# wahn/rs_pbrt

Measured on AMD Instinct MI355X. Metric: Mpath-samples/sec (whole node), higher is better.
Workload: dtype f32; 1 GPU; synthetic 1000000-triangle soup, path depth 8, sobol 256 spp, 1024x1024; tiles=16x16 tiles in Morton order dealt round-robin to the ranks (tile_chunk 1), film_reduce=none (1 GPU), devices_visible=1

## Files before the change

rs_pbrt_amd/csrc/launch_trace.h:

```cpp
uint32_t hinted_grid(uint32_t hint, uint32_t full, uint32_t per_block) {
    if (hint == 0xffffffffu) return full;
    const uint64_t need = (2ull * hint + per_block - 1) / per_block + 1;
    return (uint32_t)std::min<uint64_t>(full, need);
}
bool trace_can_overflow(const rspt_scene_s* s) {
    const size_t which = env_size("RSPT_TRACE_KERNEL", 2);
    const size_t rows = std::min<size_t>(env_size("RSPT_W4_SPILL_ROWS", RSPT_W4_SPILL), RSPT_W4_SPILL);
    return s->has_instances || (s->has_alpha && !s->w4_ok) || !(which >= 2 && s->w4_ok) || RSPT_W4_LDS + rows < RSPT_W4_MAX_STACK;
}
uint32_t trace_grid() { return grid_for((uint32_t)env_size("RSPT_TRACE_BLOCKS_PER_CU", 5)); }
#ifndef RSPT_PW_CHUNK_CAMERA_DEFAULT
#define RSPT_PW_CHUNK_CAMERA_DEFAULT 1024
#endif
#ifndef RSPT_PW_REFILL_CAMERA_DEFAULT
#define RSPT_PW_REFILL_CAMERA_DEFAULT 48
#endif
#ifndef RSPT_PW_ENTER
#define RSPT_PW_ENTER 24
#endif
struct TraceCall {
    const uint32_t* queue = nullptr; const uint32_t* count_ptr = nullptr; uint32_t count_imm = 0;
    uint32_t* cursor = nullptr;
    const rspt_ray* ra = nullptr; const rspt_ray* rb = nullptr;
    float4* oa = nullptr; float4* ob = nullptr;
    uint32_t* occ = nullptr;
    rspt_hit* hits = nullptr;
    unsigned long long* counters = nullptr; uint32_t* xcd_cursors = nullptr;
    int lane = 0;
    bool count = false;
    bool camera_launch = false;
    int force_any_q = -1;
    int force_camera_pk = -1;
    uint32_t* inst_out = nullptr;
    uint32_t queue_hint = 0xffffffffu;
};
struct TracePre { hipStream_t stream; uint32_t* ovf; uint2* spill; uint32_t pgrid; int refill, leaf; uint32_t chunk; };
TracePre trace_pre(const TraceCall& c, bool camera) {
    TracePre p; p.stream = c.lane ? g.stream2 : g.stream;
    p.ovf = g.ovf + (c.lane ? 2 * g.ovf_cap / 3 : 0);
    p.spill = g.spill + (c.lane ? g.spill_threads * RSPT_W4_SPILL : 0);
    p.pgrid = hinted_grid(c.queue_hint, pw_grid(), RSPT_PW_BLOCK);
    p.refill = (int)(camera ? env_size("RSPT_PW_REFILL_CAMERA", RSPT_PW_REFILL_CAMERA_DEFAULT) : env_size("RSPT_PW_REFILL", RSPT_PW_REFILL));
    p.leaf = (int)(camera ? env_size("RSPT_PW_LEAF_CAMERA", env_size("RSPT_PW_LEAF", RSPT_PW_LEAF)) : env_size("RSPT_PW_LEAF", RSPT_PW_LEAF));
    p.chunk = (uint32_t)std::min<size_t>(std::max<size_t>((camera ? env_size("RSPT_PW_CHUNK_CAMERA", RSPT_PW_CHUNK_CAMERA_DEFAULT) : env_size("RSPT_PW_CHUNK", RSPT_PW_CHUNK)) & ~(size_t)63, 64), 1u << 20);
    return p;
}
bool camera_packet_ok(const rspt_scene_s* s, size_t which, const uint32_t* xcur) {
    return which >= 2 && s->w4_ok && s->w4 && s->leaf_boxes && !s->has_instances && !s->has_alpha && !s->has_spheres && !(s->w4_root & RSPT_REF_LEAF) &&
           env_size("RSPT_W4_SHAPE", RSPT_W4_SHAPE_DEFAULT) == 0 && !xcur;
}
bool camera_packet_wanted(const rspt_scene_s* s, const TraceCall& c) {
    if (c.force_camera_pk >= 0) return c.force_camera_pk != 0;
    const char* e = getenv("RSPT_CAMERA_PACKET");
    if (e && *e) return atoi(e) != 0;
    return c.camera_launch && s->camera_pk_choice > 0;
}
template <bool ANY, int OUT_MODE, bool INST, bool ALPHA>
void launch_trace_v(uint32_t grid, const rspt_scene_s* s, const TraceCall& c, uint32_t* xcur) {
    const SceneDev& sc = s->dev;
    const size_t which = env_size("RSPT_TRACE_KERNEL", 2);
    const TracePre p = trace_pre(c, c.camera_launch);
    uint32_t* hi = (INST && OUT_MODE == 0 && !ANY) ? (c.inst_out ? c.inst_out : g.hit_inst) : nullptr;
    const bool special = INST || ALPHA;
    const bool anim_w4 = s->has_animated && s->w4_ok && which >= 2 && env_size("RSPT_ANIM_W4", 1) != 0 && env_size("RSPT_INSTANCE_KERNEL", 1) != 0;
    const bool slow = c.count || which == 0 || (s->has_animated && !anim_w4) || (special && (!s->w4_ok || env_size("RSPT_INSTANCE_KERNEL", 1) == 0));
    if (slow) {
        if (INST && s->has_animated)
            hipLaunchKernelGGL((k_trace<ANY, OUT_MODE, false, true, ALPHA, true>), dim3(grid), dim3(RSPT_TRACE_BLOCK), 0, p.stream, sc, s->tex, c.queue, c.count_ptr, c.count_imm, c.ra, c.rb, c.oa, c.ob, c.occ, c.hits, c.counters, hi);
        else if (c.count)
            hipLaunchKernelGGL((k_trace<ANY, OUT_MODE, true, INST, ALPHA>), dim3(grid), dim3(RSPT_TRACE_BLOCK), 0, p.stream, sc, s->tex, c.queue, c.count_ptr, c.count_imm, c.ra, c.rb, c.oa, c.ob, c.occ, c.hits, c.counters, hi);
        else
            hipLaunchKernelGGL((k_trace<ANY, OUT_MODE, false, INST, ALPHA>), dim3(grid), dim3(RSPT_TRACE_BLOCK), 0, p.stream, sc, s->tex, c.queue, c.count_ptr, c.count_imm, c.ra, c.rb, c.oa, c.ob, c.occ, c.hits, c.counters, hi);
        return;
    }
    const uint32_t pw_chunk = p.chunk | (env_size("RSPT_PW_ADAPT", 1) != 0 ? 0u : 1u);
    grid = hinted_grid(c.queue_hint, grid, RSPT_TRACE_BLOCK);
    uint32_t* n_overflow = c.cursor + 2;
    const uint32_t spill_rows = (uint32_t)std::min<size_t>(env_size("RSPT_W4_SPILL_ROWS", RSPT_W4_SPILL), RSPT_W4_SPILL);
    if constexpr (INST) {
        if (anim_w4) {
            const int pw_enter = (int)std::min<size_t>(std::max<size_t>(env_size("RSPT_PW_ENTER", RSPT_PW_ENTER), 1), 64);
            auto go = [&](auto kern) {
                hipLaunchKernelGGL(kern, dim3(p.pgrid), dim3(RSPT_PW_BLOCK), 0, p.stream, sc, s->tex, s->w4, s->big_leaves, s->w4_root, c.queue, c.count_ptr, c.count_imm, c.cursor,
                                   c.ra, c.rb, c.oa, c.ob, c.occ, c.hits, n_overflow, p.ovf, p.spill, spill_rows, p.refill, (p.leaf & 0xff) | (pw_enter << 8), s->w4_top, hi, xcur, pw_chunk);
            };
            if constexpr (ALPHA) { if (s->alpha_simple) go(k_trace_w4<ANY, OUT_MODE, true, 2, true>); else go(k_trace_w4<ANY, OUT_MODE, true, 1, true>); }
            else go(k_trace_w4<ANY, OUT_MODE, true, 0, true>);
            hipLaunchKernelGGL((k_trace_fixup<ANY, OUT_MODE, true, ALPHA, true>), dim3(grid), dim3(RSPT_TRACE_BLOCK), 0, p.stream, sc, s->tex, n_overflow, p.ovf, c.ra, c.rb, c.oa, c.ob, c.occ, c.hits, hi);
            return;
        }
    }
    if constexpr (ANY && !INST && !ALPHA) {
        const char* q_env = getenv("RSPT_ANY_Q");
        const bool use_q = c.force_any_q >= 0 ? c.force_any_q != 0 : (q_env && *q_env ? atoi(q_env) != 0 : s->any_q_choice > 0);
        if (use_q && which >= 2 && s->w4q && !(s->w4_root & RSPT_REF_LEAF) && c.ra == c.rb && env_size("RSPT_W4_SHAPE", RSPT_W4_SHAPE_DEFAULT) == 0 && !xcur && spill_rows == RSPT_W4_SPILL) {
            hipLaunchKernelGGL((k_trace_w4q<OUT_MODE>), dim3(p.pgrid), dim3(RSPT_PW_BLOCK), 0, p.stream, sc, s->w4q, s->big_leaves, s->w4_root, c.queue, c.count_ptr, c.count_imm, c.cursor,
                               c.ra, c.occ, c.hits, reinterpret_cast<uint32_t*>(p.spill), p.refill, p.leaf, s->w4_top,
                               pw_chunk | (env_size("RSPT_ANY_Q_LATE", 1) != 0 ? 2u : 0u) , s->leaf_boxes);
            return;
        }
    }
    if constexpr (!ANY && !INST && !ALPHA) {
        if (camera_packet_wanted(s, c) && camera_packet_ok(s, which, xcur)) {
            const uint32_t kgrid = hinted_grid(c.queue_hint, grid_for((uint32_t)std::min<size_t>(std::max<size_t>(env_size("RSPT_PK_BLOCKS_PER_CU", 6), 1), 8)), RSPT_PW_BLOCK);
            hipLaunchKernelGGL((k_trace_w4pk<OUT_MODE>), dim3(kgrid), dim3(RSPT_PW_BLOCK), 0, p.stream, sc, s->w4, s->big_leaves, s->w4_root, c.queue, c.count_ptr, c.count_imm, c.cursor,
                               c.ra, c.rb, c.oa, c.ob, c.hits, pw_chunk, s->leaf_boxes);
            return;
        }
    }
    if constexpr (!INST && !ALPHA) {
        const size_t shape = which >= 2 && s->w4_ok ? env_size("RSPT_W4_SHAPE", RSPT_W4_SHAPE_DEFAULT) : 0;
        if (shape == 1 || shape == 2) {
            auto go = [&](auto kern, uint32_t block, uint32_t topcap, uint32_t per_cu) -> bool {
                const size_t lds = (size_t)8 * RSPT_W4_LDS * block + (size_t)112 * topcap;
                static bool attr_set[2][2][2][3] = {};
                bool& done = attr_set[ANY ? 1 : 0][OUT_MODE ? 1 : 0][0][shape];
                static bool attr_bad[2][2][2][3] = {};
                bool& bad = attr_bad[ANY ? 1 : 0][OUT_MODE ? 1 : 0][0][shape];
                if (!done) { bad = hipFuncSetAttribute(reinterpret_cast<const void*>(kern), hipFuncAttributeMaxDynamicSharedMemorySize, (int)lds) != hipSuccess; (void)hipGetLastError(); done = true; }
                if (bad) return false;
                const uint32_t bgrid = hinted_grid(c.queue_hint, grid_for(per_cu), block);
                hipLaunchKernelGGL(kern, dim3(bgrid), dim3(block), lds, p.stream, sc, s->tex, s->w4, s->big_leaves, s->w4_root, c.queue, c.count_ptr, c.count_imm, c.cursor,
                                   c.ra, c.rb, c.oa, c.ob, c.occ, c.hits, n_overflow, p.ovf, p.spill, spill_rows, p.refill, p.leaf, s->w4_top, hi, xcur, pw_chunk);
                return true;
            };
            const bool launched = shape == 1 ? go(k_trace_w4<ANY, OUT_MODE, false, 0, false, 1024, 512>, 1024u, 512u, 1u) : go(k_trace_w4<ANY, OUT_MODE, false, 0, false, 512, 256>, 512u, 256u, 2u);
            if (launched) {
                if (trace_can_overflow(s))
                    hipLaunchKernelGGL((k_trace_fixup<ANY, OUT_MODE, INST, ALPHA>), dim3(grid), dim3(RSPT_TRACE_BLOCK), 0, p.stream, sc, s->tex, n_overflow, p.ovf, c.ra, c.rb, c.oa, c.ob, c.occ, c.hits, hi);
                return;
            }
        }
    }
    if (ALPHA && s->alpha_simple)
        hipLaunchKernelGGL((k_trace_w4<ANY, OUT_MODE, INST, ALPHA ? 2 : 0>), dim3(p.pgrid), dim3(RSPT_PW_BLOCK), 0, p.stream, sc, s->tex, s->w4, s->big_leaves, s->w4_root, c.queue, c.count_ptr, c.count_imm, c.cursor,
                           c.ra, c.rb, c.oa, c.ob, c.occ, c.hits, n_overflow, p.ovf, p.spill, spill_rows, p.refill, p.leaf, s->w4_top, hi, xcur, pw_chunk);
    else if (special || (which >= 2 && s->w4_ok))
        hipLaunchKernelGGL((k_trace_w4<ANY, OUT_MODE, INST, ALPHA ? 1 : 0>), dim3(p.pgrid), dim3(RSPT_PW_BLOCK), 0, p.stream, sc, s->tex, s->w4, s->big_leaves, s->w4_root, c.queue, c.count_ptr, c.count_imm, c.cursor,
                           c.ra, c.rb, c.oa, c.ob, c.occ, c.hits, n_overflow, p.ovf, p.spill, spill_rows, p.refill, p.leaf, s->w4_top, hi, xcur, pw_chunk);
// ... 64 lines not shown
```

rs_pbrt_amd/csrc/render_schedules.h:

```cpp
#define RSPT_LANE_ROWS(WH) {{k_lane_dl<false, false, false, WH>, k_lane_dl<false, true, false, WH>}, {k_lane_dl<true, false, false, WH>, k_lane_dl<true, true, false, WH>}, {k_lane_dl<true, false, true, WH>, k_lane_dl<true, true, true, WH>}}
typedef void (*LaneKernel)(SceneDev, TexTables, LightDistDev, RenderDev, Batch, PathBuf, const uint32_t*, LaneDesc);
const LaneKernel g_lane_dl[2][3][2] = {RSPT_LANE_ROWS(false), RSPT_LANE_ROWS(true)};
#undef RSPT_LANE_ROWS
int RenderRun::build_claimed_rows(uint32_t* n_claimed) {
    LightLazy lz;
    HIP_TRY(hipMemcpyAsync(g.look, ld_lazy->lazy, sizeof lz, hipMemcpyDeviceToHost, g.stream));
    HIP_TRY(hipStreamSynchronize(g.stream));
    memcpy(&lz, g.look, sizeof lz);
    *n_claimed = lz.n_new;
    if (lz.overflow) return fail(RSPT_E_NOMEM, "spatial light distribution: more than %u voxels were touched; raise RSPT_LIGHT_TABLE_POOL_BYTES", lz.max_rows);
    if (lz.n_new == 0) return RSPT_OK;
    const uint32_t lgrid = grid_for(4);
    hipLaunchKernelGGL(k_ld_contrib_list, dim3(lgrid), dim3(256), 0, g.stream, s->dev, ld.nvox[0], ld.nvox[1], ld.nvox[2], ld_lazy->lazy, ld_lazy->new_list, ld_lazy->func);
    hipLaunchKernelGGL(k_ld_build_list, dim3(lgrid), dim3(256), 0, g.stream, s->dev.n_lights, ld_lazy->lazy, ld_lazy->new_list, ld_lazy->func, ld_lazy->cdf, ld_lazy->func_int, ld_lazy->table);
    hipLaunchKernelGGL(k_ld_commit, dim3(1), dim3(1), 0, g.stream, ld_lazy->lazy);
    return RSPT_OK;
}
int RenderRun::tune_any(uint32_t batch_n, TraceCall c) {
    if (!s->w4q || s->any_q_choice >= 0 || getenv("RSPT_ANY_Q") || counters || batch_n < (1u << 22) || env_size("RSPT_ANY_Q_TUNE", 1) == 0) return 0;
    hipEvent_t t0 = get_event(n_ev++), t1 = get_event(n_ev++), t2 = get_event(n_ev++);
    if (hipEventRecord(t0, g.stream) != hipSuccess) return RSPT_E_HIP;
    c.force_any_q = 0;
    launch_trace<true, 0>(tgrid, s, c);
    (void)hipEventRecord(t1, g.stream);
    (void)hipMemsetAsync(c.cursor, 0, sizeof(uint32_t), g.stream);
    c.force_any_q = 1;
    launch_trace<true, 0>(tgrid, s, c);
    (void)hipEventRecord(t2, g.stream);
    if (hipEventSynchronize(t2) != hipSuccess) return RSPT_E_HIP;
    float ms_plain = 0.0f, ms_q = 0.0f;
    (void)hipEventElapsedTime(&ms_plain, t0, t1);
    (void)hipEventElapsedTime(&ms_q, t1, t2);
    s->any_q_choice = ms_q < ms_plain ? 1 : 0;
    if (getenv("RSPT_VERBOSE")) fprintf(stderr, "rspt: shadow rays of this scene: k_trace_w4<any> %.2f ms, k_trace_w4q %.2f ms on the same launch -> %s\n", ms_plain, ms_q, s->any_q_choice ? "the quantised records" : "the plain records");
    return 1;
}
int RenderRun::tune_camera(uint32_t batch_n, TraceCall c) {
    if (s->camera_pk_choice >= 0 || getenv("RSPT_CAMERA_PACKET") || counters || d->integrator != RSPT_INTEGRATOR_PATH || batch_n < (1u << 22) || env_size("RSPT_CAMERA_PACKET_TUNE", 1) == 0) return 0;
    if (!camera_packet_ok(s, env_size("RSPT_TRACE_KERNEL", 2), (c.xcd_cursors && env_size("RSPT_XCD_DEAL", 0) != 0) ? c.xcd_cursors : nullptr)) return 0;
    hipEvent_t t0 = get_event(n_ev++), t1 = get_event(n_ev++), t2 = get_event(n_ev++);
    if (hipEventRecord(t0, g.stream) != hipSuccess) return RSPT_E_HIP;
    c.force_camera_pk = 0;
    launch_trace<false, 0>(tgrid, s, c);
    (void)hipEventRecord(t1, g.stream);
    (void)hipMemsetAsync(c.cursor, 0, sizeof(uint32_t), g.stream);
    c.force_camera_pk = 1;
    launch_trace<false, 0>(tgrid, s, c);
    (void)hipEventRecord(t2, g.stream);
    if (hipEventSynchronize(t2) != hipSuccess) return RSPT_E_HIP;
    float ms_w4 = 0.0f, ms_pk = 0.0f;
    (void)hipEventElapsedTime(&ms_w4, t0, t1);
    (void)hipEventElapsedTime(&ms_pk, t1, t2);
    s->camera_pk_choice = ms_pk < ms_w4 ? 1 : 0;
    if (getenv("RSPT_VERBOSE")) fprintf(stderr, "rspt: camera rays of this scene: k_trace_w4 %.2f ms, k_trace_w4pk %.2f ms on the same launch -> %s\n", ms_w4, ms_pk, s->camera_pk_choice ? "64-ray packets" : "per-lane walks");
    return 1;
}
int RenderRun::batch_volpath(const Batch& bt, uint32_t& it) {
    int rc;
    const uint32_t dgrid = grid_for(4);
    const uint32_t null_passes = (uint32_t)env_size("RSPT_NULL_PASSES", 1024);
    const uint32_t vnd = std::min(1024u, 5u + 10u * (d->max_depth + 2u) + 128u) + 8u;
    if ((size_t)vnd * sob_bits * 4 > 64 * 1024) return fail(RSPT_E_UNSUPPORTED, "volpath: max_depth %u x %u index bits exceed the LDS Sobol' table", d->max_depth, sob_bits);
    const uint32_t vlimit = halton ? vol_dim_limit : std::min(1024u, vnd - 8u);
    hipLaunchKernelGGL(k_vol_init, dim3((bt.n + 255) / 256), dim3(256), 0, g.stream, g.vol, bt.n);
    uint32_t live = bt.n;
    for (uint32_t pass = 0; live > 0; pass++) {
        const int par = pass & 1;
        QueueCounts* cur = &g.cnt[par];
        QueueCounts* nxt = &g.cnt[par ^ 1];
        HIP_TRY(hipMemsetAsync(nxt, 0, sizeof(QueueCounts), g.stream));
        HIP_TRY(hipMemsetAsync(&g.cnt[2], 0, sizeof(QueueCounts), g.stream));
        ev_open(0, 0);
        launch_trace<false, 0>(tgrid, s, closest_call(g.pb, g.q[par][1], &cur->closest, &cur->cursor_closest, counters));
        ev_close(0, 0);
        trace_launches++;
        vol_rays += live;
        ev_open(2, 0);
        if (s->has_textures) hipLaunchKernelGGL(k_texture, dim3(dgrid), dim3(256), 0, g.stream, s->dev, s->tex, rd, g.pb, g.q[par][1], &cur->closest, (const uint32_t*)nullptr, (const BinInfo*)nullptr);
        if (ld.lazy) HIP_TRY(hipMemsetAsync(&cur->active, 0, sizeof(uint32_t), g.stream));
        hipLaunchKernelGGL(s->has_dynamic ? k_vol_shade<true> : k_vol_shade<false>, dim3(dgrid), dim3(256), halton ? 0 : vnd * sob_bits * sizeof(uint32_t), g.stream, s->dev, ld, rd, g.pb, g.vol, g.q[par][1], &cur->closest,
                           g.q[par ^ 1][1], &nxt->closest, g.q[0][2], &g.cnt[2].closest, vlimit, vnd, sob_bits, ld.lazy ? g.q[par][0] : (uint32_t*)nullptr, &cur->active);
        for (uint32_t round = 0; ld.lazy; round++) {
            uint32_t claimed = 0;
            if ((rc = build_claimed_rows(&claimed))) return rc;
            HIP_TRY(hipMemcpyAsync(g.look, cur, sizeof(QueueCounts), hipMemcpyDeviceToHost, g.stream));
            HIP_TRY(hipStreamSynchronize(g.stream));
            const uint32_t n_retry = g.look[0].active;
// ... 378 lines not shown
```

rs_pbrt_amd/csrc/trace_packet.h:

```cpp
#pragma once
#include "trace_w4.h"

namespace rspt {

#define RSPT_PK_WAVES (RSPT_PW_BLOCK / 64)
#ifdef RSPT_PK_OCC
#define RSPT_PK_ATTR __attribute__((amdgpu_waves_per_eu(RSPT_PK_OCC, RSPT_PK_OCC)))
#else
#define RSPT_PK_ATTR
#endif

typedef float pk_f4 __attribute__((ext_vector_type(4)));
typedef uint32_t pk_u2 __attribute__((ext_vector_type(2)));
RDEV float4 pk_load4(const float4* p) {
    const pk_f4 v = *reinterpret_cast<const __attribute__((address_space(4))) pk_f4*>(reinterpret_cast<uintptr_t>(p));
    return make_float4(v.x, v.y, v.z, v.w);
}
RDEV uint2 pk_load2(const uint2* p) {
    const pk_u2 v = *reinterpret_cast<const __attribute__((address_space(4))) pk_u2*>(reinterpret_cast<uintptr_t>(p));
    return make_uint2(v.x, v.y);
}

template <int OUT_MODE>
__global__ __launch_bounds__(RSPT_PW_BLOCK) RSPT_PK_ATTR void k_trace_w4pk(SceneDev sc, const Wide4Node* __restrict__ recs, const uint2* __restrict__ big_leaves, uint32_t root_ref,
                                                              const uint32_t* __restrict__ queue, const uint32_t* __restrict__ count_ptr, uint32_t count_imm, uint32_t* cursor,
                                                              const rspt_ray* __restrict__ rays_a, const rspt_ray* __restrict__ rays_b,
                                                              float4* __restrict__ out_a, float4* __restrict__ out_b, rspt_hit* __restrict__ out_hits,
                                                              uint32_t chunk ,
                                                              const float4* __restrict__ leaf_boxes) {
    __shared__ uint4 stack_s[RSPT_PK_WAVES * RSPT_W4_MAX_STACK];
    uint4* stk = stack_s + (threadIdx.x >> 6) * RSPT_W4_MAX_STACK;
    const uint32_t n = count_ptr ? *count_ptr : count_imm;
    {
        const bool adapt = !(chunk & 1u);
        chunk &= ~63u;
        const uint32_t waves = gridDim.x * (uint32_t)RSPT_PK_WAVES;
        uint32_t per = ((n + waves - 1u) / waves + 63u) & ~63u;
        if (per < 64u) per = 64u;
        if (adapt && per < chunk) chunk = per;
    }
    const uint32_t lane = __lane_id();
    const float4 root0 = sc.nodes[0], root1 = sc.nodes[1];
    uint32_t chunk_lo = 0, chunk_hi = 0;

    for (;;) {
        if (chunk_lo == chunk_hi) {
            uint32_t base = 0;
            if (lane == 0) base = atomicAdd(cursor, chunk);
            base = __builtin_amdgcn_readfirstlane(base);
            if (base >= n) break;
            chunk_lo = base;
            chunk_hi = (n - base) > chunk ? base + chunk : n;
        }
        const uint32_t qpos = chunk_lo + lane;
        const bool valid = qpos < chunk_hi;
        chunk_lo = (chunk_hi - chunk_lo) > 64u ? chunk_lo + 64u : chunk_hi;

        float ox = 0, oy = 0, oz = 0, ix = 0, iy = 0, iz = 0;
        RayShear rs{0, 0, 0, 0, 0, 0};
        float t_max = 0.0f;
        uint32_t negbits = 0, entry = 0;
        uint32_t best = RSPT_MISS;
        float bt = 0.0f, bb0 = 0.0f, bb1 = 0.0f, bb2 = 0.0f;
        bool alive = false;
        if (valid) {
            entry = queue ? queue[qpos] : qpos;
            const float4* rp = reinterpret_cast<const float4*>(((entry & RSPT_Q_MIS) ? rays_b : rays_a) + (entry & ~RSPT_Q_MIS));
            float4 r0 = rp[0], r1 = rp[1];
            ox = r0.x; oy = r0.y; oz = r0.z;
            f3 d{r0.w, r1.x, r1.y};
            t_max = r1.z;
            ix = 1.0f / d.x; iy = 1.0f / d.y; iz = 1.0f / d.z;
            negbits = (ix < 0.0f ? 1u : 0u) | (iy < 0.0f ? 2u : 0u) | (iz < 0.0f ? 4u : 0u);
            if (!(fabsf(ix) < RSPT_INF && fabsf(iy) < RSPT_INF && fabsf(iz) < RSPT_INF)) negbits |= 8u;
            rs = ray_shear(d);
            alive = box_hit(root0, root1, f3{ox, oy, oz}, f3{ix, iy, iz}, negbits & 1u, negbits & 2u, negbits & 4u, t_max);
        }

        uint64_t todo = __ballot(alive);
        while (todo) {
            const uint32_t nb = (uint32_t)__builtin_amdgcn_readlane((int)negbits, (int)(__ffsll((unsigned long long)todo) - 1));
            const uint64_t gmask = __ballot(alive && negbits == nb);
            todo &= ~gmask;
            const bool n0 = nb & 1u, n1 = nb & 2u, n2 = nb & 4u;
            uint32_t sp = 0, cur = root_ref;
            uint64_t mask = gmask;

            auto leaf_phase = [&](uint32_t offset, uint32_t n_prims, uint64_t lmask) {
                const bool in = ((lmask >> lane) & 1ull) != 0;
                const f3 o{ox, oy, oz};
                for (uint32_t i = 0; i < n_prims; i++) {
                    const uint32_t pi = offset + i;
                    const float4 a = pk_load4(sc.tris + 3 * (size_t)pi), b = pk_load4(sc.tris + 3 * (size_t)pi + 1), c = pk_load4(sc.tris + 3 * (size_t)pi + 2);
                    float t, b0, b1, b2;
                    if (in && tri_test(f3{a.x, a.y, a.z}, f3{a.w, b.x, b.y}, f3{b.z, b.w, c.x}, o, rs, t_max, &t, &b0, &b1, &b2)) {
                        t_max = t;
                        best = pi; bt = t; bb0 = b0; bb1 = b1; bb2 = b2;
                    }
                }
            };
            auto leaf_range = [&](uint32_t ref, uint32_t* offset, uint32_t* n_prims) {
                uint32_t off = ref & RSPT_W4_OFFSET_MASK, np = ((ref >> RSPT_W4_COUNT_SHIFT) & 15u) + 1u;
                if (np == 16u) {
                    const uint2 bl = pk_load2(big_leaves + off);
                    off = bl.x; np = bl.y;
                }
                *offset = off; *n_prims = np;
            };

            for (;;) {
                if (cur == RSPT_NONE) {
                    if (sp == 0) break;
                    sp--;
                    const uint4 e = stk[sp];
                    const uint32_t ref = __builtin_amdgcn_readfirstlane(e.x);
                    mask = (uint64_t)__builtin_amdgcn_readfirstlane(e.y) | ((uint64_t)__builtin_amdgcn_readfirstlane(e.z) << 32);
                    if (ref & RSPT_REF_LEAF) {
                        uint32_t offset, n_prims;
                        leaf_range(ref, &offset, &n_prims);
                        const float4 q0 = pk_load4(leaf_boxes + 2 * (size_t)offset), q1 = pk_load4(leaf_boxes + 2 * (size_t)offset + 1);
                        const bool ok = ((mask >> lane) & 1ull) != 0 && box_hit(q0, q1, f3{ox, oy, oz}, f3{ix, iy, iz}, n0, n1, n2, t_max);
                        const uint64_t lmask = __ballot(ok);
                        if (lmask) leaf_phase(offset, n_prims, lmask);
                        continue;
                    }
                    cur = ref;
                }
                const float4* pp = reinterpret_cast<const float4*>(recs + cur);
                const float4 a0 = pk_load4(pp), a1 = pk_load4(pp + 1), a2 = pk_load4(pp + 2), a3 = pk_load4(pp + 3), a4 = pk_load4(pp + 4), a5 = pk_load4(pp + 5), rf = pk_load4(pp + 6);
                cur = RSPT_NONE;
                const bool in = ((mask >> lane) & 1ull) != 0;
                bool h0, h1, h2, h3;
                float m0, m1, m2, m3;
                if (!(nb & 8u)) {
                    box_pair_hit_m(a0, a1, a2, ox, oy, oz, ix, iy, iz, t_max, &h0, &h1, &m0, &m1);
                    __builtin_amdgcn_sched_barrier(0);
                    box_pair_hit_m(a3, a4, a5, ox, oy, oz, ix, iy, iz, t_max, &h2, &h3, &m2, &m3);
                } else {
                    const f3 o{ox, oy, oz}, inv{ix, iy, iz};
                    h0 = box_hit6_m(a0.x, a1.x, a2.x, a0.z, a1.z, a2.z, o, inv, n0, n1, n2, t_max, &m0);
                    h1 = box_hit6_m(a0.y, a1.y, a2.y, a0.w, a1.w, a2.w, o, inv, n0, n1, n2, t_max, &m1);
                    h2 = box_hit6_m(a3.x, a4.x, a5.x, a3.z, a4.z, a5.z, o, inv, n0, n1, n2, t_max, &m2);
                    h3 = box_hit6_m(a3.y, a4.y, a5.y, a3.w, a4.w, a5.w, o, inv, n0, n1, n2, t_max, &m3);
                }
                h0 = h0 && in; h1 = h1 && in; h2 = h2 && in; h3 = h3 && in;
                const uint64_t s0 = __ballot(h0), s1 = __ballot(h1), s2 = __ballot(h2), s3 = __ballot(h3);
                if ((s0 | s1 | s2 | s3) == 0) continue;
                const uint32_t f0 = __builtin_amdgcn_readfirstlane(__float_as_uint(rf.x)), f1 = __builtin_amdgcn_readfirstlane(__float_as_uint(rf.y));
                const uint32_t f2 = __builtin_amdgcn_readfirstlane(__float_as_uint(rf.z)), f3w = __builtin_amdgcn_readfirstlane(__float_as_uint(rf.w));
                const bool sA = ((nb >> ((f0 >> RSPT_W4_AXIS_SHIFT) & 3u)) & 1u) != 0;
                const bool sB0 = ((nb >> ((f1 >> RSPT_W4_AXIS_SHIFT) & 3u)) & 1u) != 0;
                const bool sB1 = ((nb >> ((f2 >> RSPT_W4_AXIS_SHIFT) & 3u)) & 1u) != 0;
                const uint32_t r0 = f0 & ~RSPT_W4_AXIS_MASK, r1 = f1 & ~RSPT_W4_AXIS_MASK, r2 = f2 & ~RSPT_W4_AXIS_MASK, r3 = f3w;
                const uint32_t g0n = sB0 ? r1 : r0, g0f = sB0 ? r0 : r1, g1n = sB1 ? r3 : r2, g1f = sB1 ? r2 : r3;
                const uint64_t w0n = sB0 ? s1 : s0, w0f = sB0 ? s0 : s1, w1n = sB1 ? s3 : s2, w1f = sB1 ? s2 : s3;
                const uint32_t e0 = sA ? g1n : g0n, e1 = sA ? g1f : g0f, e2 = sA ? g0n : g1n, e3 = sA ? g0f : g1f;
                const uint64_t w0 = sA ? w1n : w0n, w1 = sA ? w1f : w0f, w2 = sA ? w0n : w1n, w3 = sA ? w0f : w1f;
                const bool p1 = w0 != 0, p2 = p1 || w1 != 0, p3 = p2 || w2 != 0;
                const bool push3 = w3 != 0 && p3, push2 = w2 != 0 && p2, push1 = w1 != 0 && p1;
                if (lane == 0) {
                    uint32_t q = sp;
                    if (push3) stk[q++] = make_uint4(e3, (uint32_t)w3, (uint32_t)(w3 >> 32), 0u);
                    if (push2) stk[q++] = make_uint4(e2, (uint32_t)w2, (uint32_t)(w2 >> 32), 0u);
                    if (push1) stk[q++] = make_uint4(e1, (uint32_t)w1, (uint32_t)(w1 >> 32), 0u);
                }
                sp += (push3 ? 1u : 0u) + (push2 ? 1u : 0u) + (push1 ? 1u : 0u);
                const uint32_t next = p1 ? e0 : (w1 != 0 ? e1 : (w2 != 0 ? e2 : e3));
                const uint64_t nmask = p1 ? w0 : (w1 != 0 ? w1 : (w2 != 0 ? w2 : w3));
                if (next & RSPT_REF_LEAF) {
                    uint32_t offset, n_prims;
                    leaf_range(next, &offset, &n_prims);
                    leaf_phase(offset, n_prims, nmask);
                } else {
                    cur = next; mask = nmask;
                }
            }
        }

        if (valid) {
            const uint32_t slot = entry & ~RSPT_Q_MIS;
            if (OUT_MODE == 0) {
                const float4 v = make_float4(__uint_as_float(best), bb0, bb1, bb2);
                if (entry & RSPT_Q_MIS) { out_b[slot] = v; asm volatile(""); }
                else out_a[slot] = v;
            } else {
                rspt_hit h;
                h.prim = best; h.t = bt; h.b0 = bb0; h.b1 = bb1; h.b2 = bb2;
                out_hits[qpos] = h;
            }
        }
    }
}

}
```

rs_pbrt_amd/csrc/tu_decl.h:

```cpp
#pragma once
#include "tile_serial.h"
#include "lane_serial.h"
#include "trace_w4.h"
#include "trace_w4q.h"
#include "trace_packet.h"

namespace rspt {

constexpr uint32_t SV_DIFFUSE = RSPT_SF_LOBE(RSPT_BXDF_LAMBERT_R) | SF_L_AREA | SF_SOBOL;
constexpr uint32_t SV_PLASTIC = SV_DIFFUSE | RSPT_SF_LOBE(RSPT_BXDF_MICROFACET_R) | SF_VERTEX;
constexpr uint32_t SV_TEXTURED = SV_PLASTIC | RSPT_SF_LOBE(RSPT_BXDF_OREN_NAYAR) | SF_TEX;
constexpr uint32_t SV_GENERIC = SF_ALL & ~SF_DYNAMIC & ~SF_ANIM;
constexpr uint32_t SV_DIFFUSE_H = (SV_DIFFUSE & ~SF_SOBOL) | SF_HALTON, SV_PLASTIC_H = (SV_PLASTIC & ~SF_SOBOL) | SF_HALTON, SV_TEXTURED_H = (SV_TEXTURED & ~SF_SOBOL) | SF_HALTON;
constexpr uint32_t SV_DYNAMIC = SF_ALL & ~SF_ANIM;
constexpr uint32_t SV_GENERIC_SPH = SV_GENERIC & ~SF_TRIS_ONLY, SV_DYNAMIC_SPH = SV_DYNAMIC & ~SF_TRIS_ONLY;
constexpr uint32_t SV_GENERIC_ML = SV_GENERIC & ~SF_NO_MAPLIGHT, SV_ALL_ML = SF_ALL & ~SF_NO_MAPLIGHT;

#define RSPT_TU_TS(I, A, M) \
    RSPT_TU_X template __global__ void k_tile_serial<I, A, M>(SceneDev, TexTables, LightDistDev, RenderDev, PathBuf, PixDesc, const TileRec*, uint32_t, uint32_t, int32_t, int32_t, float4*, float2*, uint32_t, uint32_t*);
#define RSPT_TU_TS2(I, M) RSPT_TU_TS(I, false, M) RSPT_TU_TS(I, true, M)
#define RSPT_TU_SHADE(F) RSPT_TU_X template __global__ void k_shade<F>(RSPT_SHADE_ARGS);
#define RSPT_TU_SHADE_W(F, W) RSPT_TU_X template __global__ void k_shade_w<F, W>(RSPT_SHADE_ARGS);
#define RSPT_TU_SHADE_M(F) RSPT_TU_X template __global__ void k_shade_m<F>(RSPT_SHADE_ARGS);
#define RSPT_TU_SHADE_MW(F, W) RSPT_TU_X template __global__ void k_shade_mw<F, W>(RSPT_SHADE_ARGS);
#define RSPT_TU_W4(ANY, OM, I, A) \
    RSPT_TU_X template __global__ void k_trace_w4<ANY, OM, I, A>(SceneDev, TexTables, const Wide4Node*, const uint2*, uint32_t, const uint32_t*, const uint32_t*, uint32_t, uint32_t*, const rspt_ray*, \
                                                                  const rspt_ray*, float4*, float4*, uint32_t*, rspt_hit*, uint32_t*, uint32_t*, uint2*, uint32_t, int, int, uint32_t, uint32_t*, uint32_t*, uint32_t);
#define RSPT_TU_W4A1(ANY, OM, A) \
    RSPT_TU_X template __global__ void k_trace_w4<ANY, OM, true, A, true>(SceneDev, TexTables, const Wide4Node*, const uint2*, uint32_t, const uint32_t*, const uint32_t*, uint32_t, uint32_t*, const rspt_ray*, \
                                                                           const rspt_ray*, float4*, float4*, uint32_t*, rspt_hit*, uint32_t*, uint32_t*, uint2*, uint32_t, int, int, uint32_t, uint32_t*, uint32_t*, uint32_t);
#define RSPT_TU_W4AF(ANY, OM, A) \
    RSPT_TU_X template __global__ void k_trace_fixup<ANY, OM, true, A, true>(SceneDev, TexTables, const uint32_t*, const uint32_t*, const rspt_ray*, const rspt_ray*, float4*, float4*, uint32_t*, rspt_hit*, uint32_t*);
#define RSPT_TU_W4A(ANY, OM) RSPT_TU_W4A1(ANY, OM, 0) RSPT_TU_W4AF(ANY, OM, false)
#define RSPT_TU_W4AM(ANY, OM) RSPT_TU_W4A1(ANY, OM, 1) RSPT_TU_W4A1(ANY, OM, 2) RSPT_TU_W4AF(ANY, OM, true)
#define RSPT_TU_W4B(ANY, OM, B, T) \
    RSPT_TU_X template __global__ void k_trace_w4<ANY, OM, false, 0, false, B, T>(SceneDev, TexTables, const Wide4Node*, const uint2*, uint32_t, const uint32_t*, const uint32_t*, uint32_t, uint32_t*, const rspt_ray*, \
                                                                                   const rspt_ray*, float4*, float4*, uint32_t*, rspt_hit*, uint32_t*, uint32_t*, uint2*, uint32_t, int, int, uint32_t, uint32_t*, uint32_t*, uint32_t);
#define RSPT_TU_W4SPH(ANY, A) RSPT_TU_W4SPHO(ANY, 1, A)
// ... 101 lines not shown
RSPT_TU_SHADE(SV_DYNAMIC) RSPT_TU_SHADE(SF_ALL)
#endif
#if defined(RSPT_TU_ALL) || defined(RSPT_TU_GROUP_SHADE_S)
RSPT_TU_SHADE(SV_GENERIC_SPH) RSPT_TU_SHADE(SV_DYNAMIC_SPH)
#endif
#if defined(RSPT_TU_ALL) || defined(RSPT_TU_GROUP_SHADE_L)
RSPT_TU_SHADE(SV_GENERIC_ML) RSPT_TU_SHADE(SV_ALL_ML)
#endif
#if defined(RSPT_TU_ALL) || defined(RSPT_TU_GROUP_SHADE_H)
RSPT_TU_SHADE(SV_DIFFUSE_H) RSPT_TU_SHADE_W(SV_DIFFUSE_H, 3) RSPT_TU_SHADE(SV_PLASTIC_H) RSPT_TU_SHADE_W(SV_PLASTIC_H, 3) RSPT_TU_SHADE(SV_TEXTURED_H) RSPT_TU_SHADE_W(SV_TEXTURED_H, 3)
#endif
#if defined(RSPT_TU_ALL) || defined(RSPT_TU_GROUP_SHADE_MA)
RSPT_TU_SHADE_MW(SV_DIFFUSE, 3) RSPT_TU_SHADE_MW(SV_PLASTIC, 3) RSPT_TU_SHADE_M(SV_DIFFUSE) RSPT_TU_SHADE_M(SV_PLASTIC)
#endif
#if defined(RSPT_TU_ALL) || defined(RSPT_TU_GROUP_SHADE_MB)
RSPT_TU_SHADE_M(SV_TEXTURED) RSPT_TU_SHADE_MW(SV_TEXTURED_H, 3)
#endif
#if defined(RSPT_TU_ALL) || defined(RSPT_TU_GROUP_SHADE_MC)
RSPT_TU_SHADE_M(SV_GENERIC)
#endif
#if defined(RSPT_TU_ALL) || defined(RSPT_TU_GROUP_SHADE_MH)
RSPT_TU_SHADE_MW(SV_DIFFUSE_H, 3) RSPT_TU_SHADE_MW(SV_PLASTIC_H, 3)
#endif
#if defined(RSPT_TU_ALL) || defined(RSPT_TU_GROUP_W4Q)
RSPT_TU_X template __global__ void k_trace_w4q<0>(SceneDev, const Quad4Node*, const uint2*, uint32_t, const uint32_t*, const uint32_t*, uint32_t, uint32_t*, const rspt_ray*, uint32_t*, rspt_hit*, uint32_t*, int, int, uint32_t, uint32_t, const float4*);
RSPT_TU_X template __global__ void k_trace_w4q<1>(SceneDev, const Quad4Node*, const uint2*, uint32_t, const uint32_t*, const uint32_t*, uint32_t, uint32_t*, const rspt_ray*, uint32_t*, rspt_hit*, uint32_t*, int, int, uint32_t, uint32_t, const float4*);
#endif
#if defined(RSPT_TU_ALL) || defined(RSPT_TU_GROUP_W4PK)
#define RSPT_TU_W4PK(OM) \
    RSPT_TU_X template __global__ void k_trace_w4pk<OM>(SceneDev, const Wide4Node*, const uint2*, uint32_t, const uint32_t*, const uint32_t*, uint32_t, uint32_t*, const rspt_ray*, const rspt_ray*, float4*, float4*, \
                                                        rspt_hit*, uint32_t, const float4*);
RSPT_TU_W4PK(0) RSPT_TU_W4PK(1)
#endif
#if defined(RSPT_TU_ALL) || defined(RSPT_TU_GROUP_W4)
RSPT_TU_W4_4(false, 0) RSPT_TU_W4_4(false, 1) RSPT_TU_W4_4(true, 0) RSPT_TU_W4_4(true, 1)
#endif
#if defined(RSPT_TU_ALL) || defined(RSPT_TU_GROUP_W4S)
RSPT_TU_W4_S(false, 0) RSPT_TU_W4_S(false, 1) RSPT_TU_W4_S(true, 0) RSPT_TU_W4_S(true, 1)
#endif
#if defined(RSPT_TU_ALL) || defined(RSPT_TU_GROUP_W4SPH)
RSPT_TU_W4SPH(false, 0) RSPT_TU_W4SPH(false, 1) RSPT_TU_W4SPH(false, 2) RSPT_TU_W4SPH(true, 0) RSPT_TU_W4SPH(true, 1) RSPT_TU_W4SPH(true, 2)
#endif
#if defined(RSPT_TU_ALL) || defined(RSPT_TU_GROUP_W4SPH0)
RSPT_TU_W4SPHO(false, 0, 0) RSPT_TU_W4SPHO(false, 0, 1) RSPT_TU_W4SPHO(false, 0, 2) RSPT_TU_W4SPHO(true, 0, 0) RSPT_TU_W4SPHO(true, 0, 1) RSPT_TU_W4SPHO(true, 0, 2)
#endif
#if defined(RSPT_TU_ALL) || defined(RSPT_TU_GROUP_W4A)
RSPT_TU_W4A(false, 0) RSPT_TU_W4A(false, 1) RSPT_TU_W4A(true, 0) RSPT_TU_W4A(true, 1)
#endif
#if defined(RSPT_TU_ALL) || defined(RSPT_TU_GROUP_W4AM)
RSPT_TU_W4AM(false, 0) RSPT_TU_W4AM(false, 1) RSPT_TU_W4AM(true, 0) RSPT_TU_W4AM(true, 1)
#endif
#if defined(RSPT_TU_ALL) || defined(RSPT_TU_GROUP_W4B)
RSPT_TU_W4B(false, 0, 1024, 512) RSPT_TU_W4B(false, 1, 1024, 512) RSPT_TU_W4B(true, 0, 1024, 512) RSPT_TU_W4B(true, 1, 1024, 512)
RSPT_TU_W4B(false, 0, 512, 256) RSPT_TU_W4B(false, 1, 512, 256) RSPT_TU_W4B(true, 0, 512, 256) RSPT_TU_W4B(true, 1, 512, 256)
#endif
#if defined(RSPT_TU_ALL) || defined(RSPT_TU_GROUP_REF)
RSPT_TU_REF8(false, 0) RSPT_TU_REF8(false, 1) RSPT_TU_REF8(true, 0) RSPT_TU_REF8(true, 1)
RSPT_TU_FIX4(false, 0) RSPT_TU_FIX4(false, 1) RSPT_TU_FIX4(true, 0) RSPT_TU_FIX4(true, 1)
RSPT_TU_REFA(false, 0) RSPT_TU_REFA(false, 1) RSPT_TU_REFA(true, 0) RSPT_TU_REFA(true, 1)
#endif

}
```

rs_pbrt_amd/csrc/tu_w4pk.hip:

```cpp
#include <hip/hip_runtime.h>
#include "../../include/rspt.h"
#define RSPT_TU_TEMPLATES_ONLY
#define RSPT_TU_X
#define RSPT_TU_GROUP_W4PK
#include "tu_decl.h"
```

Measured before the change: 524.8 Msamples/s.

## Add frustum-culled 64-ray packet traversal kernel for camera rays, autotuned three-way

Adds a new camera-ray trace kernel that builds a wave-wide frustum (min/max origin and inverse direction) for coherent ray groups. It tests each wide-BVH child box once per node against that frustum instead of per-ray masked box tests. The autotuner now times per-lane, packet, and frustum-packet variants and picks the fastest. The frustum test is conservative, so more nodes and leaves may be visited when rays diverge. A narrowness check falls back to the existing masked walk when the frustum would be too loose.

```diff
diff --git a/rs_pbrt_amd/csrc/launch_trace.h b/rs_pbrt_amd/csrc/launch_trace.h
--- a/rs_pbrt_amd/csrc/launch_trace.h
+++ b/rs_pbrt_amd/csrc/launch_trace.h
@@ -49,11 +49,13 @@
     return which >= 2 && s->w4_ok && s->w4 && s->leaf_boxes && !s->has_instances && !s->has_alpha && !s->has_spheres && !(s->w4_root & RSPT_REF_LEAF) &&
            env_size("RSPT_W4_SHAPE", RSPT_W4_SHAPE_DEFAULT) == 0 && !xcur;
 }
-bool camera_packet_wanted(const rspt_scene_s* s, const TraceCall& c) {
-    if (c.force_camera_pk >= 0) return c.force_camera_pk != 0;
+int camera_packet_wanted(const rspt_scene_s* s, const TraceCall& c) {
+    int v;
     const char* e = getenv("RSPT_CAMERA_PACKET");
-    if (e && *e) return atoi(e) != 0;
-    return c.camera_launch && s->camera_pk_choice > 0;
+    if (c.force_camera_pk >= 0) v = c.force_camera_pk;
+    else if (e && *e) v = atoi(e);
+    else v = c.camera_launch ? s->camera_pk_choice : 0;
+    return v <= 0 ? 0 : (v == 2 ? 2 : 1);
 }
 template <bool ANY, int OUT_MODE, bool INST, bool ALPHA>
 void launch_trace_v(uint32_t grid, const rspt_scene_s* s, const TraceCall& c, uint32_t* xcur) {
@@ -101,10 +103,11 @@
         }
     }
     if constexpr (!ANY && !INST && !ALPHA) {
-        if (camera_packet_wanted(s, c) && camera_packet_ok(s, which, xcur)) {
+        const int pk = camera_packet_wanted(s, c);
+        if (pk && camera_packet_ok(s, which, xcur)) {
             const uint32_t kgrid = hinted_grid(c.queue_hint, grid_for((uint32_t)std::min<size_t>(std::max<size_t>(env_size("RSPT_PK_BLOCKS_PER_CU", 6), 1), 8)), RSPT_PW_BLOCK);
-            hipLaunchKernelGGL((k_trace_w4pk<OUT_MODE>), dim3(kgrid), dim3(RSPT_PW_BLOCK), 0, p.stream, sc, s->w4, s->big_leaves, s->w4_root, c.queue, c.count_ptr, c.count_imm, c.cursor,
-                               c.ra, c.rb, c.oa, c.ob, c.hits, pw_chunk, s->leaf_boxes);
+            hipLaunchKernelGGL(pk == 2 ? k_trace_w4pf<OUT_MODE> : k_trace_w4pk<OUT_MODE>, dim3(kgrid), dim3(RSPT_PW_BLOCK), 0, p.stream, sc, s->w4, s->big_leaves, s->w4_root, c.queue, c.count_ptr, c.count_imm,
+                               c.cursor, c.ra, c.rb, c.oa, c.ob, c.hits, pw_chunk, s->leaf_boxes);
             return;
         }
     }
diff --git a/rs_pbrt_amd/csrc/render_schedules.h b/rs_pbrt_amd/csrc/render_schedules.h
--- a/rs_pbrt_amd/csrc/render_schedules.h
+++ b/rs_pbrt_amd/csrc/render_schedules.h
@@ -38,21 +38,22 @@
 int RenderRun::tune_camera(uint32_t batch_n, TraceCall c) {
     if (s->camera_pk_choice >= 0 || getenv("RSPT_CAMERA_PACKET") || counters || d->integrator != RSPT_INTEGRATOR_PATH || batch_n < (1u << 22) || env_size("RSPT_CAMERA_PACKET_TUNE", 1) == 0) return 0;
     if (!camera_packet_ok(s, env_size("RSPT_TRACE_KERNEL", 2), (c.xcd_cursors && env_size("RSPT_XCD_DEAL", 0) != 0) ? c.xcd_cursors : nullptr)) return 0;
-    hipEvent_t t0 = get_event(n_ev++), t1 = get_event(n_ev++), t2 = get_event(n_ev++);
-    if (hipEventRecord(t0, g.stream) != hipSuccess) return RSPT_E_HIP;
-    c.force_camera_pk = 0;
-    launch_trace<false, 0>(tgrid, s, c);
-    (void)hipEventRecord(t1, g.stream);
-    (void)hipMemsetAsync(c.cursor, 0, sizeof(uint32_t), g.stream);
-    c.force_camera_pk = 1;
-    launch_trace<false, 0>(tgrid, s, c);
-    (void)hipEventRecord(t2, g.stream);
-    if (hipEventSynchronize(t2) != hipSuccess) return RSPT_E_HIP;
-    float ms_w4 = 0.0f, ms_pk = 0.0f;
-    (void)hipEventElapsedTime(&ms_w4, t0, t1);
-    (void)hipEventElapsedTime(&ms_pk, t1, t2);
-    s->camera_pk_choice = ms_pk < ms_w4 ? 1 : 0;
-    if (getenv("RSPT_VERBOSE")) fprintf(stderr, "rspt: camera rays of this scene: k_trace_w4 %.2f ms, k_trace_w4pk %.2f ms on the same launch -> %s\n", ms_w4, ms_pk, s->camera_pk_choice ? "64-ray packets" : "per-lane walks");
+    hipEvent_t t[4] = {get_event(n_ev++), get_event(n_ev++), get_event(n_ev++), get_event(n_ev++)};
+    if (hipEventRecord(t[0], g.stream) != hipSuccess) return RSPT_E_HIP;
+    for (int k = 0; k < 3; k++) {
+        if (k) (void)hipMemsetAsync(c.cursor, 0, sizeof(uint32_t), g.stream);
+        c.force_camera_pk = k;
+        launch_trace<false, 0>(tgrid, s, c);
+        (void)hipEventRecord(t[k + 1], g.stream);
+    }
+    if (hipEventSynchronize(t[3]) != hipSuccess) return RSPT_E_HIP;
+    float ms[3] = {0.0f, 0.0f, 0.0f};
+    for (int k = 0; k < 3; k++) (void)hipEventElapsedTime(&ms[k], t[k], t[k + 1]);
+    int pick = 0;
+    for (int k = 1; k < 3; k++) if (ms[k] < ms[pick]) pick = k;
+    s->camera_pk_choice = pick;
+    static const char* const names[3] = {"per-lane walks", "64-ray packets", "64-ray packets, one frustum test per record"};
+    if (getenv("RSPT_VERBOSE")) fprintf(stderr, "rspt: camera rays of this scene: k_trace_w4 %.2f ms, k_trace_w4pk %.2f ms, k_trace_w4pf %.2f ms on the same launch -> %s\n", ms[0], ms[1], ms[2], names[pick]);
     return 1;
 }
 int RenderRun::batch_volpath(const Batch& bt, uint32_t& it) {
diff --git a/rs_pbrt_amd/csrc/trace_frustum.h b/rs_pbrt_amd/csrc/trace_frustum.h
--- /dev/null
+++ b/rs_pbrt_amd/csrc/trace_frustum.h
@@ -0,0 +1,131 @@
+#pragma once
+#include "trace_packet.h"
+
+namespace rspt {
+
+RDEV float pf_wave_min(float v) {
+    for (int m = 32; m >= 1; m >>= 1) v = fminf(v, __shfl_xor(v, m));
+    return __uint_as_float(__builtin_amdgcn_readfirstlane(__float_as_uint(v)));
+}
+RDEV float pf_wave_max(float v) {
+    for (int m = 32; m >= 1; m >>= 1) v = fmaxf(v, __shfl_xor(v, m));
+    return __uint_as_float(__builtin_amdgcn_readfirstlane(__float_as_uint(v)));
+}
+
+struct PfFrustum {
+    static constexpr bool frustum = true;
+    template <class LeafPhase, class LeafRange>
+    static RDEV bool walk(const Wide4Node* __restrict__ recs, const float4* __restrict__ leaf_boxes, float4 root0, float4 root1, uint32_t root_ref, uint2* stk, uint32_t lane, uint32_t nb, uint64_t gmask,
+                          float ox, float oy, float oz, float ix, float iy, float iz, float& t_max, LeafPhase& leaf_phase, LeafRange& leaf_range) {
+        const float widen = 1.0f + 2.0f * gamma_n(3);
+        const bool n0 = nb & 1u, n1 = nb & 2u, n2 = nb & 4u;
+        const bool ing = ((gmask >> lane) & 1ull) != 0;
+        const float o_lo[3] = {pf_wave_min(ing ? ox : RSPT_INF), pf_wave_min(ing ? oy : RSPT_INF), pf_wave_min(ing ? oz : RSPT_INF)};
+        const float o_hi[3] = {pf_wave_max(ing ? ox : -RSPT_INF), pf_wave_max(ing ? oy : -RSPT_INF), pf_wave_max(ing ? oz : -RSPT_INF)};
+        const float inv_lo[3] = {pf_wave_min(ing ? ix : RSPT_INF), pf_wave_min(ing ? iy : RSPT_INF), pf_wave_min(ing ? iz : RSPT_INF)};
+        const float inv_hi[3] = {pf_wave_max(ing ? ix : -RSPT_INF), pf_wave_max(ing ? iy : -RSPT_INF), pf_wave_max(ing ? iz : -RSPT_INF)};
+        float tmax_bound = pf_wave_max(ing ? t_max : -RSPT_INF);
+        {
+            const float ext[3] = {root0.w - root0.x, root1.x - root0.y, root1.y - root0.z};
+            bool narrow = true;
+            for (int a = 0; a < 3; a++) {
+                const bool neg = (nb >> a) & 1u;
+                narrow = narrow && (o_hi[a] - o_lo[a]) * 16.0f <= ext[a] && (neg ? inv_lo[a] >= 1.5f * inv_hi[a] : inv_hi[a] <= 1.5f * inv_lo[a]);
+            }
+            if (!narrow) return false;
+        }
+        uint32_t sp = 0, cur = root_ref;
+
+        auto leaf = [&](uint32_t ref) {
+            uint32_t offset, n_prims;
+            leaf_range(ref, &offset, &n_prims);
+            const float4 q0 = pk_load4(leaf_boxes + 2 * (size_t)offset), q1 = pk_load4(leaf_boxes + 2 * (size_t)offset + 1);
+            const bool ok = ing && box_hit(q0, q1, f3{ox, oy, oz}, f3{ix, iy, iz}, n0, n1, n2, t_max);
+            const uint64_t lmask = __ballot(ok);
+            RSPT_PK_COUNT_ADD(1);
+            if (lmask == 0) return;
+            const float before = t_max;
+            leaf_phase(offset, n_prims, lmask);
+            if (__ballot(t_max != before)) tmax_bound = pf_wave_max(ing ? t_max : -RSPT_INF);
+        };
+
+        for (;;) {
+            if (cur == RSPT_NONE) {
+                if (sp == 0) break;
+                sp--;
+                const uint2 e = stk[sp];
+                const uint32_t ref = __builtin_amdgcn_readfirstlane(e.x);
+                const float le = __uint_as_float(__builtin_amdgcn_readfirstlane(e.y));
+                if (!(le < tmax_bound)) continue;
+                if (ref & RSPT_REF_LEAF) {
+                    leaf(ref);
+                    continue;
+                }
+                cur = ref;
+            }
+            RSPT_PK_COUNT_ADD(0);
+            const char* base = reinterpret_cast<const char*>(recs + cur);
+            const float4 rf = pk_load4(reinterpret_cast<const float4*>(base) + 6);
+            cur = RSPT_NONE;
+            uint32_t lk = lane;
+            asm volatile("" : "+v"(lk));
+            const uint32_t boff = (lk & 2u) * 24u + (lk & 1u) * 4u;
+            const float* bp = reinterpret_cast<const float*>(base + boff);
+            const float ax = bp[0] - o_hi[0], bx = bp[2] - o_lo[0], ay = bp[4] - o_hi[1], by = bp[6] - o_lo[1], az = bp[8] - o_hi[2], bz = bp[10] - o_lo[2];
+            const float pxa = ax * inv_lo[0], pxb = ax * inv_hi[0], pxc = bx * inv_lo[0], pxd = bx * inv_hi[0];
+            const float pya = ay * inv_lo[1], pyb = ay * inv_hi[1], pyc = by * inv_lo[1], pyd = by * inv_hi[1];
+            const float pza = az * inv_lo[2], pzb = az * inv_hi[2], pzc = bz * inv_lo[2], pzd = bz * inv_hi[2];
+            const float lx = fminf(fminf(fminf(pxa, pxb), pxc), pxd), ux = fmaxf(fmaxf(fmaxf(pxa, pxb), pxc), pxd);
+            const float ly = fminf(fminf(fminf(pya, pyb), pyc), pyd), uy = fmaxf(fmaxf(fmaxf(pya, pyb), pyc), pyd);
+            const float lz = fminf(fminf(fminf(pza, pzb), pzc), pzd), uz = fmaxf(fmaxf(fmaxf(pza, pzb), pzc), pzd);
+            const float L = fmaxf(fmaxf(lx, ly), lz);
+            const float U = fminf(fminf(ux, uy), uz) * widen;
+            const bool taken = (L <= U) && (L < tmax_bound) && (U > 0.0f);
+            uint32_t f0 = __builtin_amdgcn_readfirstlane(__float_as_uint(rf.x)), f1 = __builtin_amdgcn_readfirstlane(__float_as_uint(rf.y));
+            uint32_t f2 = __builtin_amdgcn_readfirstlane(__float_as_uint(rf.z)), f3w = __builtin_amdgcn_readfirstlane(__float_as_uint(rf.w));
+            asm volatile("" : "+s"(f0), "+s"(f1), "+s"(f2), "+s"(f3w));
+            const uint32_t bits = (uint32_t)__ballot(taken) & 15u;
+            if (bits == 0) continue;
+            const bool sA = ((nb >> ((f0 >> RSPT_W4_AXIS_SHIFT) & 3u)) & 1u) != 0;
+            const bool sB0 = ((nb >> ((f1 >> RSPT_W4_AXIS_SHIFT) & 3u)) & 1u) != 0;
+            const bool sB1 = ((nb >> ((f2 >> RSPT_W4_AXIS_SHIFT) & 3u)) & 1u) != 0;
+            const uint32_t r0 = f0 & ~RSPT_W4_AXIS_MASK, r1 = f1 & ~RSPT_W4_AXIS_MASK, r2 = f2 & ~RSPT_W4_AXIS_MASK, r3 = f3w;
+            const uint32_t lb = __float_as_uint(L);
+            const uint32_t l0 = (uint32_t)__builtin_amdgcn_readlane((int)lb, 0), l1 = (uint32_t)__builtin_amdgcn_readlane((int)lb, 1);
+            const uint32_t l2 = (uint32_t)__builtin_amdgcn_readlane((int)lb, 2), l3 = (uint32_t)__builtin_amdgcn_readlane((int)lb, 3);
+            const bool s0 = bits & 1u, s1 = bits & 2u, s2 = bits & 4u, s3 = bits & 8u;
+            const uint32_t g0n = sB0 ? r1 : r0, g0f = sB0 ? r0 : r1, g1n = sB1 ? r3 : r2, g1f = sB1 ? r2 : r3;
+            const uint32_t d0n = sB0 ? l1 : l0, d0f = sB0 ? l0 : l1, d1n = sB1 ? l3 : l2, d1f = sB1 ? l2 : l3;
+            const bool w0n = sB0 ? s1 : s0, w0f = sB0 ? s0 : s1, w1n = sB1 ? s3 : s2, w1f = sB1 ? s2 : s3;
+            const uint32_t e0 = sA ? g1n : g0n, e1 = sA ? g1f : g0f, e2 = sA ? g0n : g1n, e3 = sA ? g0f : g1f;
+            const uint32_t d1 = sA ? d1f : d0f, d2 = sA ? d0n : d1n, d3 = sA ? d0f : d1f;
+            const bool w0 = sA ? w1n : w0n, w1 = sA ? w1f : w0f, w2 = sA ? w0n : w1n, w3 = sA ? w0f : w1f;
+            const bool p1 = w0, p2 = p1 || w1, p3 = p2 || w2;
+            const bool push3 = w3 && p3, push2 = w2 && p2, push1 = w1 && p1;
+            if (lane == 0) {
+                uint32_t q = sp;
+                if (push3) stk[q++] = make_uint2(e3, d3);
+                if (push2) stk[q++] = make_uint2(e2, d2);
+                if (push1) stk[q++] = make_uint2(e1, d1);
+            }
+            sp += (push3 ? 1u : 0u) + (push2 ? 1u : 0u) + (push1 ? 1u : 0u);
+            const uint32_t next = p1 ? e0 : (w1 ? e1 : (w2 ? e2 : e3));
+            if (next & RSPT_REF_LEAF) leaf(next);
+            else cur = next;
+        }
+        return true;
+    }
+};
+
+template <int OUT_MODE>
+__global__ __launch_bounds__(RSPT_PW_BLOCK) RSPT_PK_ATTR void k_trace_w4pf(SceneDev sc, const Wide4Node* __restrict__ recs, const uint2* __restrict__ big_leaves, uint32_t root_ref,
+                                                              const uint32_t* __restrict__ queue, const uint32_t* __restrict__ count_ptr, uint32_t count_imm, uint32_t* cursor,
+                                                              const rspt_ray* __restrict__ rays_a, const rspt_ray* __restrict__ rays_b,
+                                                              float4* __restrict__ out_a, float4* __restrict__ out_b, rspt_hit* __restrict__ out_hits,
+                                                              uint32_t chunk, const float4* __restrict__ leaf_boxes) {
+    __shared__ uint4 stack_s[RSPT_PK_WAVES * RSPT_W4_MAX_STACK];
+    pk_trace_body<OUT_MODE, PfFrustum>(stack_s + (threadIdx.x >> 6) * RSPT_W4_MAX_STACK, sc, recs, big_leaves, root_ref, queue, count_ptr, count_imm, cursor, rays_a, rays_b, out_a, out_b, out_hits,
+                                       chunk, leaf_boxes);
+}
+
+}
diff --git a/rs_pbrt_amd/csrc/trace_packet.h b/rs_pbrt_amd/csrc/trace_packet.h
--- a/rs_pbrt_amd/csrc/trace_packet.h
+++ b/rs_pbrt_amd/csrc/trace_packet.h
@@ -21,15 +21,26 @@
     return make_uint2(v.x, v.y);
 }
 
-template <int OUT_MODE>
-__global__ __launch_bounds__(RSPT_PW_BLOCK) RSPT_PK_ATTR void k_trace_w4pk(SceneDev sc, const Wide4Node* __restrict__ recs, const uint2* __restrict__ big_leaves, uint32_t root_ref,
-                                                              const uint32_t* __restrict__ queue, const uint32_t* __restrict__ count_ptr, uint32_t count_imm, uint32_t* cursor,
-                                                              const rspt_ray* __restrict__ rays_a, const rspt_ray* __restrict__ rays_b,
-                                                              float4* __restrict__ out_a, float4* __restrict__ out_b, rspt_hit* __restrict__ out_hits,
-                                                              uint32_t chunk ,
-                                                              const float4* __restrict__ leaf_boxes) {
-    __shared__ uint4 stack_s[RSPT_PK_WAVES * RSPT_W4_MAX_STACK];
-    uint4* stk = stack_s + (threadIdx.x >> 6) * RSPT_W4_MAX_STACK;
+#ifdef RSPT_PK_COUNT
+static __device__ unsigned long long g_pk_count[3];
+#define RSPT_PK_COUNT_ADD(i) do { if (__lane_id() == 0) atomicAdd(&g_pk_count[i], 1ull); } while (0)
+#else
+#define RSPT_PK_COUNT_ADD(i) do { } while (0)
+#endif
+
+struct PkMaskedOnly {
+    static constexpr bool frustum = false;
+    template <class LeafPhase, class LeafRange>
+    static RDEV bool walk(const Wide4Node*, const float4*, float4, float4, uint32_t, uint2*, uint32_t, uint32_t, uint64_t, float, float, float, float, float, float, float&, LeafPhase&, LeafRange&) { return false; }
+};
+
+template <int OUT_MODE, class FR>
+RDEV void pk_trace_body(uint4* stk, const SceneDev& sc, const Wide4Node* __restrict__ recs, const uint2* __restrict__ big_leaves, uint32_t root_ref,
+                        const uint32_t* __restrict__ queue, const uint32_t* __restrict__ count_ptr, uint32_t count_imm, uint32_t* cursor,
+                        const rspt_ray* __restrict__ rays_a, const rspt_ray* __restrict__ rays_b,
+                        float4* __restrict__ out_a, float4* __restrict__ out_b, rspt_hit* __restrict__ out_hits,
+                        uint32_t chunk ,
+                        const float4* __restrict__ leaf_boxes) {
     const uint32_t n = count_ptr ? *count_ptr : count_imm;
     {
         const bool adapt = !(chunk & 1u);
@@ -78,6 +89,7 @@
         }
 
         uint64_t todo = __ballot(alive);
+        if (todo) RSPT_PK_COUNT_ADD(2);
         while (todo) {
             const uint32_t nb = (uint32_t)__builtin_amdgcn_readlane((int)negbits, (int)(__ffsll((unsigned long long)todo) - 1));
             const uint64_t gmask = __ballot(alive && negbits == nb);
@@ -108,6 +120,9 @@
                 *offset = off; *n_prims = np;
             };
 
+            if (FR::frustum && !(nb & 8u) &&
+                FR::walk(recs, leaf_boxes, root0, root1, root_ref, reinterpret_cast<uint2*>(stk), lane, nb, gmask, ox, oy, oz, ix, iy, iz, t_max, leaf_phase, leaf_range))
+                continue;
             for (;;) {
                 if (cur == RSPT_NONE) {
                     if (sp == 0) break;
@@ -121,18 +136,20 @@
                         const float4 q0 = pk_load4(leaf_boxes + 2 * (size_t)offset), q1 = pk_load4(leaf_boxes + 2 * (size_t)offset + 1);
                         const bool ok = ((mask >> lane) & 1ull) != 0 && box_hit(q0, q1, f3{ox, oy, oz}, f3{ix, iy, iz}, n0, n1, n2, t_max);
                         const uint64_t lmask = __ballot(ok);
+                        RSPT_PK_COUNT_ADD(1);
                         if (lmask) leaf_phase(offset, n_prims, lmask);
                         continue;
                     }
                     cur = ref;
                 }
+                RSPT_PK_COUNT_ADD(0);
                 const float4* pp = reinterpret_cast<const float4*>(recs + cur);
                 const float4 a0 = pk_load4(pp), a1 = pk_load4(pp + 1), a2 = pk_load4(pp + 2), a3 = pk_load4(pp + 3), a4 = pk_load4(pp + 4), a5 = pk_load4(pp + 5), rf = pk_load4(pp + 6);
                 cur = RSPT_NONE;
                 const bool in = ((mask >> lane) & 1ull) != 0;
                 bool h0, h1, h2, h3;
                 float m0, m1, m2, m3;
-                if (!(nb & 8u)) {
+                if (!FR::frustum && !(nb & 8u)) {
                     box_pair_hit_m(a0, a1, a2, ox, oy, oz, ix, iy, iz, t_max, &h0, &h1, &m0, &m1);
                     __builtin_amdgcn_sched_barrier(0);
                     box_pair_hit_m(a3, a4, a5, ox, oy, oz, ix, iy, iz, t_max, &h2, &h3, &m2, &m3);
@@ -192,4 +209,15 @@
     }
 }
 
-}
+template <int OUT_MODE>
+__global__ __launch_bounds__(RSPT_PW_BLOCK) RSPT_PK_ATTR void k_trace_w4pk(SceneDev sc, const Wide4Node* __restrict__ recs, const uint2* __restrict__ big_leaves, uint32_t root_ref,
+                                                              const uint32_t* __restrict__ queue, const uint32_t* __restrict__ count_ptr, uint32_t count_imm, uint32_t* cursor,
+                                                              const rspt_ray* __restrict__ rays_a, const rspt_ray* __restrict__ rays_b,
+                                                              float4* __restrict__ out_a, float4* __restrict__ out_b, rspt_hit* __restrict__ out_hits,
+                                                              uint32_t chunk, const float4* __restrict__ leaf_boxes) {
+    __shared__ uint4 stack_s[RSPT_PK_WAVES * RSPT_W4_MAX_STACK];
+    pk_trace_body<OUT_MODE, PkMaskedOnly>(stack_s + (threadIdx.x >> 6) * RSPT_W4_MAX_STACK, sc, recs, big_leaves, root_ref, queue, count_ptr, count_imm, cursor, rays_a, rays_b, out_a, out_b, out_hits,
+                                          chunk, leaf_boxes);
+}
+
+}
diff --git a/rs_pbrt_amd/csrc/tu_decl.h b/rs_pbrt_amd/csrc/tu_decl.h
--- a/rs_pbrt_amd/csrc/tu_decl.h
+++ b/rs_pbrt_amd/csrc/tu_decl.h
@@ -4,6 +4,7 @@
 #include "trace_w4.h"
 #include "trace_w4q.h"
 #include "trace_packet.h"
+#include "trace_frustum.h"
 
 namespace rspt {
 
@@ -171,6 +172,12 @@
                                                         rspt_hit*, uint32_t, const float4*);
 RSPT_TU_W4PK(0) RSPT_TU_W4PK(1)
 #endif
+#if defined(RSPT_TU_ALL) || defined(RSPT_TU_GROUP_W4PF)
+#define RSPT_TU_W4PF(OM) \
+    RSPT_TU_X template __global__ void k_trace_w4pf<OM>(SceneDev, const Wide4Node*, const uint2*, uint32_t, const uint32_t*, const uint32_t*, uint32_t, uint32_t*, const rspt_ray*, const rspt_ray*, float4*, float4*, \
+                                                        rspt_hit*, uint32_t, const float4*);
+RSPT_TU_W4PF(0) RSPT_TU_W4PF(1)
+#endif
 #if defined(RSPT_TU_ALL) || defined(RSPT_TU_GROUP_W4)
 RSPT_TU_W4_4(false, 0) RSPT_TU_W4_4(false, 1) RSPT_TU_W4_4(true, 0) RSPT_TU_W4_4(true, 1)
 #endif
diff --git a/rs_pbrt_amd/csrc/tu_w4pf.hip b/rs_pbrt_amd/csrc/tu_w4pf.hip
--- /dev/null
+++ b/rs_pbrt_amd/csrc/tu_w4pf.hip
@@ -0,0 +1,13 @@
+#include <hip/hip_runtime.h>
+#include "../../include/rspt.h"
+#define RSPT_TU_TEMPLATES_ONLY
+#define RSPT_TU_X
+#define RSPT_TU_GROUP_W4PF
+#include "tu_decl.h"
+#ifdef RSPT_PK_COUNT
+extern "C" int rspt_pk_count_pf(unsigned long long* out3) {
+    unsigned long long zero[3] = {0, 0, 0};
+    if (hipDeviceSynchronize() != hipSuccess || hipMemcpyFromSymbol(out3, HIP_SYMBOL(rspt::g_pk_count), sizeof zero) != hipSuccess) return -1;
+    return hipMemcpyToSymbol(HIP_SYMBOL(rspt::g_pk_count), zero, sizeof zero) == hipSuccess ? 0 : -1;
+}
+#endif
diff --git a/rs_pbrt_amd/csrc/tu_w4pk.hip b/rs_pbrt_amd/csrc/tu_w4pk.hip
--- a/rs_pbrt_amd/csrc/tu_w4pk.hip
+++ b/rs_pbrt_amd/csrc/tu_w4pk.hip
@@ -4,3 +4,10 @@
 #define RSPT_TU_X
 #define RSPT_TU_GROUP_W4PK
 #include "tu_decl.h"
+#ifdef RSPT_PK_COUNT
+extern "C" int rspt_pk_count_pk(unsigned long long* out3) {
+    unsigned long long zero[3] = {0, 0, 0};
+    if (hipDeviceSynchronize() != hipSuccess || hipMemcpyFromSymbol(out3, HIP_SYMBOL(rspt::g_pk_count), sizeof zero) != hipSuccess) return -1;
+    return hipMemcpyToSymbol(HIP_SYMBOL(rspt::g_pk_count), zero, sizeof zero) == hipSuccess ? 0 : -1;
+}
+#endif
```

New measurement: 534.1 Msamples/s (median of 6 runs). 1.02x the previous value.
